# scientificcomputing/networks_fenicsx

Hardware: NVIDIA B200
Metric: tree-network assemble+solve DOFs/s (higher is better)
Workload: dtype f64

## Files before the change

networks_fenicsx_b200/csrc/ctx.cuh:

```cuda
#pragma once

#include <cuda_runtime.h>

#include <cstdarg>
#include <cstdint>
#include <cstdio>
#include <cstring>
#include <string>
#include <vector>

#include "../../include/nxfx_b200.h"

namespace nxfx {

constexpr int kTileRows = 256;
constexpr int kTileCap = 2048;
constexpr int kThreads = 256;

template <typename T>
struct DevBuf {
  T* p = nullptr;
  size_t n = 0;
  cudaError_t alloc(size_t count) {
    release();
// ... 72 lines not shown
  bool bottom_factored = false;
  int32_t n_nodes = 0, E = 0, gdim = 0, N = 0, n_bif = 0, n_inc = 0;
  int64_t nv = 0, nc = 0, nq = 0, poff = 0, loff = 0, ndofs = 0, nnz = 0;
  nxfx::DevBuf<double> x;
  nxfx::DevBuf<double> pos_stage;
  nxfx::DevBuf<int4> slot_uvl;
  nxfx::DevBuf<int2> slot_uv;
  nxfx::DevBuf<uint32_t> bif_in_bits;
  nxfx::DevBuf<int32_t> slot_edge, edge_slot, edge_u, edge_v, bif_ptr, bif_inc;
  nxfx::DevBuf<int32_t> rowptr, colidx, tile_base;
  bool pipe_ok = false;
  bool generic = false;
  nxfx::DevBuf<int32_t> gen_src_id, gen_bptr, gen_bid;
  nxfx::DevBuf<double> gen_src_coef, gen_bcoef, gen_cell_h;
  nxfx::Condensation cond;
  std::vector<nxfx::MatState*> mats;
  nxfx::MatState* cur = nullptr;
  int64_t next_mat_id = 1;
  bool pc_unscaled = false;
  int64_t pc_mat = -1;
  std::vector<int32_t> edge_slot_h;
  nxfx::TreeSchedule tree;
  nxfx::DevBuf<double> edge_g, edge_c, edge_fn;
  nxfx::DevBuf<double> work;
  nxfx::DevBuf<double> work2;
  nxfx::DevBuf<double> scal;
  nxfx::DevBuf<unsigned int> ticket;
  double* scal_h = nullptr;
  double* scal_h_dev = nullptr;
  bool pdl_coop_refused = false;
  int32_t n_shared = 0;
  nxfx::DevBuf<int32_t> shared_lm;
  std::vector<int32_t> shared_lm_h;
  nxfx::DevBuf<int32_t> top_sh_pos;
  nxfx::DevBuf<int32_t> top_sh_idx;
  nxfx::DevBuf<double> lam_weight, lam_nonshared;
  nxfx::DevBuf<double> p_nonshared;
  nxfx::PeerComm comm;
  double* mirror_h = nullptr;
  cudaStream_t side = nullptr;
  cudaEvent_t ev_x = nullptr;
  nxfx::DevBuf<double> e2e_pbc, e2e_b, e2e_x;
};

namespace nxfx {

// ... 34 lines not shown
```

networks_fenicsx_b200/csrc/nxfx_b200.cu:

```cuda

#include <cub/device/device_scan.cuh>

#include <algorithm>
#include <atomic>
#include <chrono>
#include <cmath>
#include <cstdlib>

#include "assemble.cuh"
#include "ctx.cuh"
#include "condense.cuh"
#include "generic.cuh"
#include "precond.cuh"
#include "spmv.cuh"

using namespace nxfx;

namespace {

constexpr int kScalPartials = 8 * kMaxPartials;
constexpr int kScalSlots = 1024;

Net make_net(const nxfx_ctx* c) {
  Net g;
// ... 227 lines not shown
  return NXFX_OK;
}

int do_residual(nxfx_ctx* ctx, const double* b, const double* x, double* r, double* norm2_d, bool pdl = false) {
  const int ntiles = (int)cdiv(ctx->ndofs, kTileRows);
  if (ctx->comm.ready) {
    NXFX_REQUIRE(ctx, ctx->pipe_ok && ctx->lam_nonshared.p, "the fused partitioned residual needs the pipelined SpMV and nxfx_set_shared");
    const int grid = std::min(ntiles, ctx->sm_count * kPipeBlocksPerSM);
    cudaLaunchConfig_t cfg = {};
    cfg.gridDim = dim3(grid);
    cfg.blockDim = dim3(kTileRows);
    cfg.dynamicSmemBytes = kPipeSmem;
    cfg.stream = ctx->stream;
    cudaLaunchAttribute attr[1];
    attr[0].id = cudaLaunchAttributeProgrammaticStreamSerialization;
    attr[0].val.programmaticStreamSerializationAllowed = 1;
    cfg.attrs = attr;
    cfg.numAttrs = pdl ? 1 : 0;
    NXFX_CUDA(ctx, cudaLaunchKernelEx(&cfg, spmv_pipe_kernel<3>, (int)ctx->ndofs, ntiles, (const int32_t*)ctx->rowptr.p,
                                      (const int32_t*)ctx->colidx.p, (const double*)ctx->cur->vals.p,
                                      (const int32_t*)ctx->tile_base.p, x, r, b, ctx->scal.p, ctx->ticket.p, norm2_d,
                                      (int)ctx->loff, (const double*)ctx->lam_nonshared.p, (const double*)ctx->lam_weight.p,
                                      make_peer(ctx, 1), (const int32_t*)ctx->shared_lm.p, (int)ctx->n_shared,
                                      ctx->comm.lam_scratch.p));
    ctx->launches++;
    return NXFX_OK;
  }
  if (ctx->pipe_ok && !pdl) {
    const int grid = std::min(ntiles, ctx->sm_count * kPipeBlocksPerSM);
    NXFX_LAUNCH(ctx, spmv_pipe_kernel<1>, grid, kTileRows, kPipeSmem, (int)ctx->ndofs, ntiles,
                ctx->rowptr.p, ctx->colidx.p, ctx->cur->vals.p, ctx->tile_base.p, x, r, b, ctx->scal.p,
                ctx->ticket.p, norm2_d);
    return NXFX_OK;
  }
  if (ctx->pipe_ok) {
    const int grid = std::min(ntiles, ctx->sm_count * kPipeBlocksPerSM);
    cudaLaunchConfig_t cfg = {};
    cfg.gridDim = dim3(grid);
    cfg.blockDim = dim3(kTileRows);
    cfg.dynamicSmemBytes = kPipeSmem;
    cfg.stream = ctx->stream;
    cudaLaunchAttribute attr[1];
    attr[0].id = cudaLaunchAttributeProgrammaticStreamSerialization;
    attr[0].val.programmaticStreamSerializationAllowed = 1;
    cfg.attrs = attr;
    cfg.numAttrs = 1;
    NXFX_CUDA(ctx, cudaLaunchKernelEx(&cfg, spmv_pipe_kernel<1>, (int)ctx->ndofs, ntiles, (const int32_t*)ctx->rowptr.p,
                                      (const int32_t*)ctx->colidx.p, (const double*)ctx->cur->vals.p,
                                      (const int32_t*)ctx->tile_base.p, x, r, b, ctx->scal.p, ctx->ticket.p, norm2_d, 0,
                                      (const double*)nullptr, (const double*)nullptr, PeerDev{}, (const int32_t*)nullptr, 0,
                                      (double*)nullptr));
    ctx->launches++;
    return NXFX_OK;
  }
  const int grid = std::min(ntiles, kMaxPartials);
  NXFX_LAUNCH(ctx, spmv_kernel<1>, grid, kTileRows, 0, (int)ctx->ndofs, ntiles, ctx->rowptr.p,
              ctx->colidx.p, ctx->cur->vals.p, x, r, b, ctx->scal.p, ctx->ticket.p, norm2_d);
  return NXFX_OK;
}

template <int K>
int launch_multi_dot(nxfx_ctx* ctx, int n, const double* A, size_t stride, const double* w, double* out) {
  NXFX_LAUNCH(ctx, multi_dot_kernel<K>, vec_grid(ctx, n), kThreads, 0, n, A, stride, w, ctx->scal.p,
              ctx->ticket.p, out);
  return NXFX_OK;
}

int do_multi_dot(nxfx_ctx* ctx, int n, int k, const double* A, size_t stride, const double* w, double* out) {
  int j = 0;
  while (j < k) {
    const int m = std::min(8, k - j);
    const double* Aj = A + (size_t)j * stride;
    int rc = NXFX_OK;
    switch (m) {
      case 8: rc = launch_multi_dot<8>(ctx, n, Aj, stride, w, out + j); break;
      case 7: rc = launch_multi_dot<7>(ctx, n, Aj, stride, w, out + j); break;
      case 6: rc = launch_multi_dot<6>(ctx, n, Aj, stride, w, out + j); break;
      case 5: rc = launch_multi_dot<5>(ctx, n, Aj, stride, w, out + j); break;
      case 4: rc = launch_multi_dot<4>(ctx, n, Aj, stride, w, out + j); break;
      case 3: rc = launch_multi_dot<3>(ctx, n, Aj, stride, w, out + j); break;
// ... 145 lines not shown

int cond_backward_local(nxfx_ctx* ctx, double* z, bool add) {
  Net g = make_net(ctx);
  CondDev c = make_cond(ctx);
  TreeDev t = make_tree(ctx);
  const int nb = ctx->tree.n_chunks - 1;
  if (ctx->n_bif > 0 && nb > 0) NXFX_LAUNCH(ctx, btree_sweep_kernel<2>, nb, 1024, 0, t, c, 0);
  const int grid = (int)cdiv((int64_t)ctx->E + ctx->n_bif, kCondThreads);
  if (add) NXFX_LAUNCH(ctx, cond_backsub_kernel<true>, grid, kCondThreads, 0, g, t, c, z);
  else NXFX_LAUNCH(ctx, cond_backsub_kernel<false>, grid, kCondThreads, 0, g, t, c, z);
  return NXFX_OK;
}

int do_cond_apply(nxfx_ctx* ctx, const double* r, double* z, bool add) {
  NXFX_REQUIRE(ctx, ctx->pc_ready, "pc_setup has not been run");
  int rc = cond_forward_local(ctx, r, nullptr);
  if (rc) return rc;
  if (ctx->n_bif > 0) NXFX_LAUNCH(ctx, btree_sweep_kernel<3>, 1, 1024, 0, make_tree(ctx), make_cond(ctx), ctx->tree.n_chunks - 1);
  return cond_backward_local(ctx, z, add);
}

bool n1_kernels(const nxfx_ctx* ctx) { return ctx->N == 1 && ctx->tree.fast_ok; }

int check_aligned(nxfx_ctx* ctx, const double* r, const double* z = nullptr) {
  NXFX_REQUIRE(ctx, (reinterpret_cast<uintptr_t>(r) & 15) == 0 && (reinterpret_cast<uintptr_t>(z) & 15) == 0,
               "vectors must be 16-byte aligned");
  return NXFX_OK;
}

int node_diag(nxfx_ctx* ctx, bool bif) {
  if (n1_kernels(ctx)) {
    if (bif) NXFX_LAUNCH(ctx, bif_diag_n1_kernel, (int)cdiv(ctx->n_bif, kThreads), kThreads, 0, make_net(ctx), make_tree(ctx), ctx->cur->cell_rh.p);
    return NXFX_OK;
  }
  NXFX_LAUNCH(ctx, edge_conductance_kernel, (int)cdiv(ctx->E, kThreads), kThreads, 0, ctx->E, ctx->N, ctx->cur->cell_rh.p, ctx->edge_g.p);
  if (bif) NXFX_LAUNCH(ctx, bif_diag_kernel, (int)cdiv(ctx->n_bif, kThreads), kThreads, 0, make_net(ctx), make_tree(ctx), ctx->edge_g.p);
  return NXFX_OK;
}

int node_rhs(nxfx_ctx* ctx, const double* r, bool bif) {
  Net g = make_net(ctx);
  TreeDev t = make_tree(ctx);
  if (n1_kernels(ctx)) {
    if (bif) NXFX_LAUNCH(ctx, bif_rhs_n1_kernel, (int)cdiv(ctx->n_bif, kThreads), kThreads, 0, g, t, r, ctx->cur->cell_rh.p, ctx->lam_weight.p);
    return NXFX_OK;
  }
  NXFX_LAUNCH(ctx, edge_condense_kernel<false>, (int)cdiv(ctx->E, kThreads), kThreads, 0, g, ctx->cur->cell_rh.p, r,
              ctx->edge_c.p, ctx->edge_fn.p, nullptr);
  if (bif)
    NXFX_LAUNCH(ctx, bif_rhs_kernel<false>, (int)cdiv(ctx->n_bif, kThreads), kThreads, 0, g, t, r, ctx->edge_g.p, ctx->edge_c.p,
                ctx->edge_fn.p, ctx->lam_weight.p);
  return NXFX_OK;
}

int edge_backsub(nxfx_ctx* ctx, const double* r, double* z, bool add, bool pdl = false) {
  Net g = make_net(ctx);
  TreeDev t = make_tree(ctx);
  const double* cell_rh = ctx->cur->cell_rh.p;
  const int grid = (int)cdiv((int64_t)ctx->E + ctx->n_bif, kThreads);
  if (!n1_kernels(ctx)) {
    if (add) NXFX_LAUNCH(ctx, edge_backsub_kernel<true>, grid, kThreads, 0, g, t, cell_rh, r, ctx->edge_g.p, ctx->edge_c.p, z);
    else NXFX_LAUNCH(ctx, edge_backsub_kernel<false>, grid, kThreads, 0, g, t, cell_rh, r, ctx->edge_g.p, ctx->edge_c.p, z);
    return NXFX_OK;
  }
  if (!pdl) {
    if (add) NXFX_LAUNCH(ctx, edge_backsub_n1_kernel<true>, grid, kThreads, 0, g, t, cell_rh, r, z);
    else NXFX_LAUNCH(ctx, edge_backsub_n1_kernel<false>, grid, kThreads, 0, g, t, cell_rh, r, z);
    return NXFX_OK;
  }
  cudaLaunchConfig_t cfg = {};
  cfg.gridDim = dim3((unsigned)grid);
  cfg.blockDim = dim3(kThreads);
  cfg.stream = ctx->stream;
  cudaLaunchAttribute attr[1];
  attr[0].id = cudaLaunchAttributeProgrammaticStreamSerialization;
  attr[0].val.programmaticStreamSerializationAllowed = 1;
  cfg.attrs = attr;
  cfg.numAttrs = 1;
  if (add) NXFX_CUDA(ctx, cudaLaunchKernelEx(&cfg, edge_backsub_n1_kernel<true>, g, t, cell_rh, r, z));
  else NXFX_CUDA(ctx, cudaLaunchKernelEx(&cfg, edge_backsub_n1_kernel<false>, g, t, cell_rh, r, z));
  ctx->launches++;
  return NXFX_OK;
}

int do_pc_setup(nxfx_ctx* ctx) {
  NXFX_REQUIRE(ctx, is_assembled(ctx), "assemble the matrix before pc_setup");
  if (ctx->generic) return do_cond_setup(ctx);
  NXFX_REQUIRE(ctx, ctx->tree.set, "nxfx_set_tree_schedule has not been called");
  const bool n1 = n1_kernels(ctx);
  int rc;
  if (!n1 && (rc = node_diag(ctx, ctx->n_bif > 0))) return rc;
  if (ctx->n_bif > 0 && (rc = tree_pass(ctx, true, nullptr, n1))) return rc;
  mark_factored(ctx);
  return NXFX_OK;
}

bool can_fuse_setup(const nxfx_ctx* ctx) {
  return !ctx->generic && ctx->tree.set && ctx->tree.fast_ok && ctx->tree.coop_fs_ok && ctx->n_bif > 0 &&
         ctx->tree.n_chunks > 1 && (!ctx->lam_weight.p || ctx->comm.ready) && ctx->cur->acc_count == 1;
}

int do_pc_setup_apply(nxfx_ctx* ctx, const double* r, double* z, bool add = false) {
  NXFX_REQUIRE(ctx, is_assembled(ctx), "assemble the matrix before pc_setup");
  const bool n1 = n1_kernels(ctx);
  if (n1) {
    int rc = check_aligned(ctx, r, z);
    if (rc) return rc;
  }
  auto& s = ctx->tree;
  Net g = make_net(ctx);
  TreeDev t = make_tree(ctx);
  FusedN1 fin{g, r, ctx->cur->cell_rh.p, ctx->lam_weight.p};
  unsigned int* tk = ctx->ticket.p + 1;
  unsigned int* fl = ctx->ticket.p + 2;
  unsigned int ep = ++s.epoch;
  int nb = s.n_chunks - 1;
  PeerDev pc = make_peer(ctx, 0);
  if (!n1) {
    NXFX_LAUNCH(ctx, edge_condense_kernel<true>, (int)cdiv(ctx->E, kThreads), kThreads, 0, g, ctx->cur->cell_rh.p, r,
                ctx->edge_c.p, ctx->edge_fn.p, ctx->edge_g.p);
    NXFX_LAUNCH(ctx, bif_rhs_kernel<true>, (int)cdiv(ctx->n_bif, kThreads), kThreads, 0, g, t, r, ctx->edge_g.p,
                ctx->edge_c.p, ctx->edge_fn.p, ctx->lam_weight.p);
    fin.r = nullptr;
    fin.cell_rh = nullptr;
  }
// ... 3 lines not shown
  cfg.blockDim = dim3(kTreeThreads);
  cfg.dynamicSmemBytes = tree_smem_bytes_fs(s.cap);
  cfg.stream = ctx->stream;
  cudaLaunchAttribute attr[2];
  attr[0].id = cudaLaunchAttributeCooperative;
  attr[0].val.cooperative = 1;
  attr[1].id = cudaLaunchAttributeProgrammaticStreamSerialization;
  attr[1].val.programmaticStreamSerializationAllowed = 1;
  cfg.attrs = attr;
  cfg.numAttrs = ctx->pdl_coop_refused ? 1 : 2;
  const bool multi = gb < nb;
  auto kern = pc.nranks > 1 ? (multi ? tree_factor_solve_coop_kernel<true, true> : tree_factor_solve_coop_kernel<true, false>)
                            : (multi ? tree_factor_solve_coop_kernel<false, true> : tree_factor_solve_coop_kernel<false, false>);
  cudaError_t le = cudaLaunchKernelEx(&cfg, kern, t, nb, tk, fl, ep, fin, pc);
  if (le != cudaSuccess && cfg.numAttrs == 2) {
    cudaGetLastError();
    ctx->pdl_coop_refused = true;
    cfg.numAttrs = 1;
    le = cudaLaunchKernelEx(&cfg, kern, t, nb, tk, fl, ep, fin, pc);
  }
  NXFX_CUDA(ctx, le);
  ctx->launches++;
  mark_factored(ctx);
  return edge_backsub(ctx, r, z, add, true);
}

int do_pc_apply(nxfx_ctx* ctx, int pc_type, const double* r, double* z, bool add = false) {
  const int n = (int)ctx->ndofs;
  if (pc_type == NXFX_PC_NETWORK_SCHUR && ctx->cur->acc_count > 1 && !ctx->pc_unscaled) {
    const size_t ld = vec_stride(ctx);
    if (ctx->work2.n < 2 * ld) {
      NXFX_CUDA(ctx, cudaStreamSynchronize(ctx->stream));
      NXFX_CUDA(ctx, ctx->work2.alloc(2 * ld));
    }
    const double inv_k = 1.0 / (double)ctx->cur->acc_count;
    double* rs = ctx->work2.p;
    double* zs = ctx->work2.p + ld;
    NXFX_LAUNCH(ctx, scale_tail_kernel<false>, vec_grid(ctx, n), kThreads, 0, n, (int)ctx->poff, inv_k, r, rs);
    ctx->pc_unscaled = true;
    const int rc = do_pc_apply(ctx, pc_type, rs, zs, false);
    ctx->pc_unscaled = false;
    if (rc) return rc;
    if (add) NXFX_LAUNCH(ctx, scale_tail_kernel<true>, vec_grid(ctx, n), kThreads, 0, n, (int)ctx->poff, inv_k, zs, z);
    else NXFX_LAUNCH(ctx, scale_tail_kernel<false>, vec_grid(ctx, n), kThreads, 0, n, (int)ctx->poff, inv_k, zs, z);
    return NXFX_OK;
  }
  if (add && pc_type != NXFX_PC_NETWORK_SCHUR) {
    int rc = ensure_work(ctx, 3);
    if (rc) return rc;
    double* tmp = ctx->work.p + 2 * vec_stride(ctx);
// ... 3 lines not shown
  }
  if (ctx->comm.ready) {
    NXFX_REQUIRE(ctx, pc_type == NXFX_PC_NETWORK_SCHUR && can_fuse_setup(ctx),
                 "the fused partitioned solve needs a forest schedule that fits the cooperative kernel and pc_type lu");
    return do_pc_setup_apply(ctx, r, z, add);
  }
  if (pc_type == NXFX_PC_NONE) {
    NXFX_CUDA(ctx, cudaMemcpyAsync(z, r, n * sizeof(double), cudaMemcpyDeviceToDevice, ctx->stream));
    return NXFX_OK;
  }
  if (pc_type == NXFX_PC_JACOBI_FLUX) {
    NXFX_LAUNCH(ctx, jacobi_flux_kernel, (int)cdiv(n, kThreads), kThreads, 0, n, (int)ctx->nq,
                ctx->rowptr.p, ctx->colidx.p, ctx->cur->vals.p, r, z);
    return NXFX_OK;
  }
  NXFX_REQUIRE(ctx, ctx->pc_ready, "pc_setup has not been run");
  if (ctx->generic) return do_cond_apply(ctx, r, z, add);
  const bool n1 = n1_kernels(ctx);
  int rc;
  if (n1 && (rc = check_aligned(ctx, r, z))) return rc;
  const bool fuse = n1 && ctx->n_bif > 0 && ctx->tree.coop_ok && ctx->tree.n_chunks > 1 && !ctx->lam_weight.p;
  if ((rc = node_rhs(ctx, r, ctx->n_bif > 0 && !fuse))) return rc;
  if (ctx->n_bif > 0 && (rc = tree_pass(ctx, false, r, fuse))) return rc;
  return edge_backsub(ctx, r, z, add);
}

int factor_bottom(nxfx_ctx* ctx) {
  if (ctx->generic) return cond_factor_local(ctx);
  int rc = node_diag(ctx, true);
  if (rc) return rc;
  const int nb = ctx->tree.n_chunks - 1;
  if (nb > 0) NXFX_LAUNCH(ctx, tree_factor_kernel, nb, kTreeThreads, tree_smem_bytes(ctx->tree.cap), make_tree(ctx), nb, ctx->ticket.p + 1, 0,
                          (FusedN1{make_net(ctx), nullptr, nullptr}));
  return NXFX_OK;
}

int forward_bottom(nxfx_ctx* ctx, const double* r) {
  if (ctx->generic) return cond_forward_local(ctx, r, ctx->lam_weight.p);
  int rc = node_rhs(ctx, r, true);
  if (rc) return rc;
  const int nb = ctx->tree.n_chunks - 1;
  if (nb > 0) NXFX_LAUNCH(ctx, tree_solve_kernel<kTreeUp>, nb, kTreeThreads, tree_smem_bytes(ctx->tree.cap), make_tree(ctx), nb, ctx->ticket.p + 1, 0);
  return NXFX_OK;
}

template <bool FACTOR, int PHASE>
int top_split(nxfx_ctx* ctx, double* buf) {
// ... 54 lines not shown
bool poll_norms_enabled() {
  static const bool on = [] { const char* e = std::getenv("NXFX_POLL_NORMS"); return !(e && e[0] == '0'); }();
  return on;
}

void push_history(nxfx_solve_info* info, double v) {
  if (info->history_len < NXFX_HISTORY_LEN) info->history[info->history_len++] = v;
}

int mirror_copy(nxfx_ctx* ctx, const double* x) {
  if (!ctx->mirror_h) return NXFX_OK;
  NXFX_CUDA(ctx, cudaEventRecord(ctx->ev_x, ctx->stream));
  NXFX_CUDA(ctx, cudaStreamWaitEvent(ctx->side, ctx->ev_x, 0));
  NXFX_CUDA(ctx, cudaMemcpyAsync(ctx->mirror_h, x, (size_t)ctx->ndofs * sizeof(double), cudaMemcpyDeviceToHost, ctx->side));
  return NXFX_OK;
}

int solve_preonly(nxfx_ctx* ctx, const double* b, double* x, const nxfx_solve_opts* o, nxfx_solve_info* info,
                  bool fused_setup) {
  int rc = ensure_work(ctx, 3);
  if (rc) return rc;
  double* r = ctx->work.p;
  const int steps = std::max(0, std::min(o->refine_steps, 32));
  if ((rc = fused_setup ? do_pc_setup_apply(ctx, b, x) : do_pc_apply(ctx, o->pc_type, b, x, false))) return rc;
  if ((rc = mirror_copy(ctx, x))) return rc;
  info->iterations = 1;
  if (steps == 0 && !o->final_residual) {
    NXFX_CUDA(ctx, cudaStreamSynchronize(ctx->stream));
    info->rhs_norm = info->residual_norm = -1.0;
    info->converged = 1;
    return NXFX_OK;
  }
  const double rt = o->refine_rtol > 0.0 ? o->refine_rtol : 0.0;
  int applied = 0;
  while (true) {
    const bool lazy = ctx->pipe_ok;
    volatile double* nh = ctx->scal_h;
    const bool poll = poll_norms_enabled();
    if (poll) { ctx->scal_h[0] = kNormSentinel(); ctx->scal_h[1] = kNormSentinel(); }
    if ((rc = do_residual(ctx, b, x, lazy ? nullptr : r, ctx->scal_h_dev, true))) return rc;
    bool arrived = false;
    if (poll) {
      const auto t0 = std::chrono::steady_clock::now();
      for (unsigned spin = 0;; ++spin) {
        if (!is_norm_sentinel(nh[0]) && !is_norm_sentinel(nh[1])) { arrived = true; break; }
        if ((spin & 255u) == 255u && std::chrono::steady_clock::now() - t0 > std::chrono::microseconds(1500)) break;
      }
      std::atomic_thread_fence(std::memory_order_acquire);
    }
    if (!arrived) NXFX_CUDA(ctx, cudaStreamSynchronize(ctx->stream));
    info->rhs_norm = std::sqrt(ctx->scal_h[1]);
    info->residual_norm = std::sqrt(ctx->scal_h[0]);
    push_history(info, info->residual_norm);
    const bool good = std::isfinite(info->residual_norm) && info->residual_norm <= rt * info->rhs_norm;
    if (applied >= steps || (good && rt > 0.0) || !std::isfinite(info->residual_norm)) break;
    if (lazy && (rc = do_residual(ctx, b, x, r, slot(ctx, 0)))) return rc;
    if ((rc = do_pc_apply(ctx, o->pc_type, r, x, true))) return rc;
    if ((rc = mirror_copy(ctx, x))) return rc;
    ++applied;
    if (applied >= steps && !o->final_residual) break;
  }
  info->iterations = 1 + applied;
  const double tol = std::max(o->rtol * info->rhs_norm, o->atol);
// ... 79 lines not shown
    }
  }
  info->iterations = its;
  info->converged = std::isfinite(info->residual_norm) && info->residual_norm <= tol;
  return NXFX_OK;
}

int setup_spmv_tiles(nxfx_ctx* ctx) {
  const int n = (int)ctx->ndofs;
  const int ntiles = (int)cdiv(n, kTileRows);
  NXFX_CUDA(ctx, ctx->tile_base.alloc((size_t)ntiles + 2));
  int32_t* max_tile = reinterpret_cast<int32_t*>(ctx->ticket.p);
  NXFX_LAUNCH(ctx, tile_base_kernel, (int)cdiv(ntiles + 1, kThreads), kThreads, 0, n, ntiles, ctx->rowptr.p,
              ctx->tile_base.p, max_tile);
  int32_t max_tile_h = 0;
  NXFX_CUDA(ctx, cudaMemcpyAsync(&max_tile_h, max_tile, sizeof(int32_t), cudaMemcpyDeviceToHost, ctx->stream));
  NXFX_CUDA(ctx, cudaMemsetAsync(ctx->ticket.p, 0, sizeof(unsigned int), ctx->stream));
  NXFX_CUDA(ctx, cudaStreamSynchronize(ctx->stream));
  ctx->pipe_ok = max_tile_h + 8 <= kPipeCap;
  if (ctx->pipe_ok) {
    NXFX_CUDA(ctx, cudaFuncSetAttribute(spmv_pipe_kernel<0>, cudaFuncAttributeMaxDynamicSharedMemorySize, (int)kPipeSmem));
    NXFX_CUDA(ctx, cudaFuncSetAttribute(spmv_pipe_kernel<1>, cudaFuncAttributeMaxDynamicSharedMemorySize, (int)kPipeSmem));
    NXFX_CUDA(ctx, cudaFuncSetAttribute(spmv_pipe_kernel<2>, cudaFuncAttributeMaxDynamicSharedMemorySize, (int)kPipeSmem));
  }
  return NXFX_OK;
}

}

extern "C" {

int nxfx_abi_version(void) { return NXFX_ABI_VERSION; }

int nxfx_create(nxfx_ctx** out, int device) {
  if (!out) return NXFX_ERR_INVALID;
  *out = nullptr;
  int count = 0;
  cudaError_t e = cudaGetDeviceCount(&count);
  if (e != cudaSuccess || device < 0 || device >= count) return NXFX_ERR_CUDA;
  if (cudaSetDevice(device) != cudaSuccess) return NXFX_ERR_CUDA;
  auto* ctx = new nxfx_ctx();
  ctx->device = device;
  cudaDeviceProp prop;
  if (cudaGetDeviceProperties(&prop, device) == cudaSuccess) ctx->sm_count = prop.multiProcessorCount;
  cudaEventCreate(&ctx->ev0);
  cudaEventCreate(&ctx->ev1);
// ... 137 lines not shown
  int rc;
  if ((rc = upload(ctx, ctx->pos_stage, node_pos, (size_t)n_nodes * gdim))) return rc;
  if ((rc = upload(ctx, ctx->edge_u, edge_u, (size_t)E))) return rc;
  if ((rc = upload(ctx, ctx->edge_v, edge_v, (size_t)E))) return rc;
  if ((rc = upload(ctx, ctx->edge_slot, edge_slot, (size_t)E))) return rc;
  if ((rc = upload(ctx, ctx->slot_edge, slot_edge.data(), (size_t)E))) return rc;
  if ((rc = upload(ctx, ctx->slot_uvl, uvl.data(), (size_t)E))) return rc;
  std::vector<int2> uv((size_t)E);
  for (int64_t s = 0; s < E; ++s) uv[s] = make_int2(uvl[s].x, uvl[s].y);
  if ((rc = upload(ctx, ctx->slot_uv, uv.data(), (size_t)E))) return rc;
  std::vector<uint32_t> in_bits((size_t)(n_inc + 31) / 32 + 1, 0u);
  for (int32_t k = 0; k < n_inc; ++k)
    if (bif_inc[k] & 1) in_bits[k >> 5] |= 1u << (k & 31);
  if ((rc = upload(ctx, ctx->bif_in_bits, in_bits.data(), in_bits.size()))) return rc;
  DevBuf<int32_t> node_lm_d;
  if ((rc = upload(ctx, node_lm_d, node_lm, (size_t)n_nodes))) return rc;
  if ((rc = upload(ctx, ctx->bif_ptr, bif_ptr, (size_t)n_bif + 1))) return rc;
  if ((rc = upload(ctx, ctx->bif_inc, bif_inc, (size_t)n_inc))) return rc;
  NXFX_CUDA(ctx, ctx->x.alloc((size_t)nv * 4));
  NXFX_CUDA(ctx, cudaMemsetAsync(ctx->x.p, 0, (size_t)nv * 4 * sizeof(double), ctx->stream));
  NXFX_CUDA(ctx, ctx->edge_g.alloc((size_t)E));
  NXFX_CUDA(ctx, ctx->edge_c.alloc((size_t)E));
  NXFX_CUDA(ctx, ctx->edge_fn.alloc((size_t)E));
  if ((rc = ensure_scal(ctx))) return rc;
  if ((rc = build_vertices(ctx))) return rc;
  NXFX_LAUNCH(ctx, tag_lm_kernel, (int)cdiv(n_nodes, kThreads), kThreads, 0, n_nodes, node_lm_d.p, ctx->x.p);
  NXFX_CUDA(ctx, cudaStreamSynchronize(ctx->stream));
  ctx->has_network = true;
  return NXFX_OK;
}

int nxfx_update_node_positions(nxfx_ctx* ctx, const double* node_pos) {
  if (!ctx) return NXFX_ERR_INVALID;
  NXFX_REQUIRE(ctx, ctx->has_network && node_pos, "no network / null input");
  NXFX_CUDA(ctx, cudaMemcpyAsync(ctx->pos_stage.p, node_pos, (size_t)ctx->n_nodes * ctx->gdim * sizeof(double),
                                 cudaMemcpyHostToDevice, ctx->stream));
  return build_vertices(ctx);
}

int nxfx_get_sizes(const nxfx_ctx* ctx, int64_t* nv, int64_t* nc, int64_t* ndofs, int64_t* nnz) {
  if (!ctx || !ctx->has_network) return NXFX_ERR_INVALID;
  if (nv) *nv = ctx->nv;
  if (nc) *nc = ctx->nc;
  if (ndofs) *ndofs = ctx->ndofs;
  if (nnz) *nnz = ctx->nnz;
  return NXFX_OK;
// ... 804 lines not shown
```

networks_fenicsx_b200/csrc/precond.cuh:

```cuda
#pragma once

#include "assemble.cuh"
#include "peer.cuh"
#include "spmv.cuh"

namespace nxfx {

struct TreeDev {
  const int32_t* __restrict__ t_of_bif;
  const int32_t* __restrict__ bif_of_t;
  const int32_t* __restrict__ t_parent;
  const int32_t* __restrict__ t_pedge;
  const int32_t* __restrict__ t_pslot;
  const int32_t* __restrict__ t_cptr;
  const int32_t* __restrict__ t_cidx;
  const int32_t* __restrict__ chunk_lptr;
  const int32_t* __restrict__ lvl_ptr;
  const int32_t* __restrict__ chunk_desc;
  const int32_t* __restrict__ t_inc_ptr;
  const int2* __restrict__ t_inc;
  double* diag0;
  double* tg;
  double* d;
  double* gd;
// ... 1078 lines not shown
  const int n = t.t_of_bif[i];
  t.diag0[n] = s;
  const int pe = t.t_pslot[n];
  t.tg[n] = pe >= 0 ? 1.0 / cell_rh[pe] : 0.0;
}

__global__ void __launch_bounds__(kThreads)
bif_rhs_n1_kernel(Net g, TreeDev t, const double* __restrict__ r, const double* __restrict__ cell_rh,
                  const double* __restrict__ lam_weight) {
  const int i = blockIdx.x * blockDim.x + threadIdx.x;
  if (i >= g.n_bif) return;
  double s = lam_weight ? -lam_weight[i] * r[g.loff + i] : -r[g.loff + i];
  for (int k = g.bif_ptr[i]; k < g.bif_ptr[i + 1]; ++k) {
    const int inc = g.bif_inc[k], e = inc >> 1;
    const int slot = g.edge_slot[e];
    const double2 rq = *reinterpret_cast<const double2*>(r + 2 * (size_t)slot);
    const double rp = r[g.poff + e], rh = cell_rh[slot];
    const double gc = (1.0 / rh) * (rq.x + rq.y) - 0.5 * rp;
    s += (inc & 1) ? (rp + gc) : -gc;
  }
  t.r[t.t_of_bif[i]] = s;
}

template <bool ADD>
__global__ void __launch_bounds__(kThreads)
edge_backsub_n1_kernel(Net g, TreeDev t, const double* __restrict__ cell_rh, const double* __restrict__ r,
                       double* __restrict__ z) {
  asm volatile("griddepcontrol.launch_dependents;");
  const int idx = blockIdx.x * blockDim.x + threadIdx.x;
  if (idx >= g.E) {
    asm volatile("griddepcontrol.wait;" ::: "memory");
    const int i = idx - g.E;
    if (i < g.n_bif) { if (ADD) z[g.loff + i] += t.lam_nat[i]; else z[g.loff + i] = t.lam_nat[i]; }
    return;
  }
  const int slot = idx;
  const int4 uv = g.slot_uvl[slot];
  const int e = g.slot_edge[slot];
  const double2 rq = *reinterpret_cast<const double2*>(r + 2 * (size_t)slot);
  const double rp = r[g.poff + e], rh = cell_rh[slot];
  asm volatile("griddepcontrol.wait;" ::: "memory");
  const double lu = uv.z >= 0 ? t.lam_nat[uv.z] : 0.0;
  const double lv = uv.w >= 0 ? t.lam_nat[uv.w] : 0.0;
  const double c = (rq.x + rq.y) - 0.5 * rh * rp;
  const double q0 = (c + lu - lv) / rh;
  const double q1 = q0 + rp;
  const double p = lu + rq.x - rh * (q0 * kThird + q1 * kSixth);
  double2* zq = reinterpret_cast<double2*>(z + 2 * (size_t)slot);
  if (ADD) {
    const double2 o = *zq;
    *zq = make_double2(o.x + q0, o.y + q1);
    z[g.poff + e] += p;
  } else {
    *zq = make_double2(q0, q1);
    z[g.poff + e] = p;
  }
}

__global__ void __launch_bounds__(kThreads)
pack_shared_kernel(int n_shared, int loff, const int32_t* __restrict__ shared_lm,
                   const double* __restrict__ v, double* __restrict__ buf) {
  const int i = blockIdx.x * blockDim.x + threadIdx.x;
  if (i < n_shared) buf[i] = v[loff + shared_lm[i]];
}

__global__ void __launch_bounds__(kThreads)
residual_finish_kernel(int n_shared, int loff, const int32_t* __restrict__ shared_lm,
                       const double* __restrict__ buf, double* __restrict__ r, double* __restrict__ nrm_out) {
  __shared__ double red[kThreads / 32];
  double acc = 0.0;
  for (int i = threadIdx.x; i < n_shared; i += blockDim.x) {
    const double v = buf[i];
    r[loff + shared_lm[i]] = v;
    acc += v * v;
  }
  acc = warp_sum(acc);
  if ((threadIdx.x & 31) == 0) red[threadIdx.x >> 5] = acc;
  __syncthreads();
// ... 24 lines not shown
```

networks_fenicsx_b200/csrc/spmv.cuh:

```cuda
#pragma once

#include "ctx.cuh"
#include "peer.cuh"

namespace nxfx {

constexpr int kEntriesPerThread = kTileCap / kTileRows;
constexpr int kMaxPartials = 4096;

__device__ __forceinline__ double warp_sum(double v) {
#pragma unroll
  for (int o = 16; o > 0; o >>= 1) v += __shfl_down_sync(0xffffffffu, v, o);
  return v;
}

template <int THREADS>
__device__ __forceinline__ double block_sum(double v, double* red ) {
  v = warp_sum(v);
  const int lane = threadIdx.x & 31, w = threadIdx.x >> 5;
  if (lane == 0) red[w] = v;
  __syncthreads();
  double s = 0.0;
  if (w == 0) {
    s = lane < THREADS / 32 ? red[lane] : 0.0;
    s = warp_sum(s);
  }
  __syncthreads();
  return s;
}

template <int THREADS, int K>
__device__ __forceinline__ bool finish_partials(double (&mine)[K], double* partial, int nblocks,
                                                unsigned int* ticket, double* out, double* red) {
  __shared__ bool last;
  if (threadIdx.x == 0) {
#pragma unroll
    for (int k = 0; k < K; ++k) partial[(size_t)k * kMaxPartials + blockIdx.x] = mine[k];
    __threadfence();
    const unsigned int t = atomicAdd(ticket, 1u);
    last = (t == (unsigned int)nblocks - 1);
  }
  __syncthreads();
  if (!last) return false;
  __threadfence();
#pragma unroll
  for (int k = 0; k < K; ++k) {
    double s = 0.0;
    for (int i = threadIdx.x; i < nblocks; i += THREADS)
      s += ((volatile double*)partial)[(size_t)k * kMaxPartials + i];
    s = block_sum<THREADS>(s, red);
    if (threadIdx.x == 0) out[k] = s;
  }
  if (threadIdx.x == 0) *ticket = 0u;
  return true;
}

template <int MODE>
__global__ void __launch_bounds__(kTileRows)
spmv_kernel(int n, int ntiles, const int32_t* __restrict__ rowptr,
            const int32_t* __restrict__ colidx, const double* __restrict__ vals,
            const double* __restrict__ x, double* __restrict__ y, const double* __restrict__ b,
            double* partial, unsigned int* ticket, double* norm2_out) {
  __shared__ double sm[kTileCap];
  __shared__ int srow[kTileRows + 1];
  __shared__ double red[kTileRows / 32];
  double nrm = 0.0, nrb = 0.0;
  for (int tile = blockIdx.x; tile < ntiles; tile += gridDim.x) {
    const int r0 = tile * kTileRows;
    const int nr = min(kTileRows, n - r0);
    if (threadIdx.x <= nr) srow[threadIdx.x] = rowptr[r0 + threadIdx.x];
// ... 93 lines not shown
  }
}

__global__ void __launch_bounds__(kThreads)
tile_base_kernel(int n, int ntiles, const int32_t* __restrict__ rowptr, int32_t* __restrict__ tile_base,
                 int32_t* __restrict__ max_tile_nnz) {
  const int t = blockIdx.x * blockDim.x + threadIdx.x;
  if (t > ntiles) return;
  const int r = min(t * kTileRows, n);
  const int b = rowptr[r];
  tile_base[t] = b;
  if (t < ntiles) atomicMax(max_tile_nnz, rowptr[min(r + kTileRows, n)] - b);
}

template <int MODE>
__global__ void __launch_bounds__(kTileRows)
spmv_pipe_kernel(int n, int ntiles, const int32_t* __restrict__ rowptr,
                 const int32_t* __restrict__ colidx, const double* __restrict__ vals,
                 const int32_t* __restrict__ tile_base, const double* __restrict__ x,
                 double* __restrict__ y, const double* __restrict__ b, double* partial,
                 unsigned int* ticket, double* norm2_out, int loff = 0,
                 const double* __restrict__ w_r = nullptr, const double* __restrict__ w_b = nullptr,
                 PeerDev pc = PeerDev{}, const int32_t* __restrict__ shared_lm = nullptr, int n_shared = 0,
                 double* lam_scratch = nullptr) {
  extern __shared__ __align__(128) unsigned char smem_raw[];
  SpmvStage* st = reinterpret_cast<SpmvStage*>(smem_raw);
  uint64_t* full = reinterpret_cast<uint64_t*>(smem_raw + kStages * sizeof(SpmvStage));
  __shared__ double red[kTileRows / 32];
  const int tid = threadIdx.x;
  if (tid == 0) {
    for (int s = 0; s < kStages; ++s) mbar_init(full + s, 1);
    asm volatile("fence.mbarrier_init.release.cluster;" ::: "memory");
    asm volatile("fence.proxy.async.shared::cta;" ::: "memory");
  }
  __syncthreads();
  const uint64_t stream_policy = l2_evict_first_policy();
  auto issue = [&](int tile, int s) {
    const int r0 = tile * kTileRows;
    const int nr = min(kTileRows, n - r0);
    const int sb = tile_base[tile], se = tile_base[tile + 1];
    const int s4 = sb & ~3;
    const int cnt4 = ((se + 3) & ~3) - s4;
    const uint32_t rbytes = (uint32_t)(((nr + 1) * 4 + 15) & ~15);
    mbar_expect_tx(full + s, (uint32_t)cnt4 * 12u + rbytes);
    if (cnt4 > 0) {
      bulk_g2s_stream(st[s].vals, vals + s4, (uint32_t)cnt4 * 8u, full + s, stream_policy);
      bulk_g2s_stream(st[s].cols, colidx + s4, (uint32_t)cnt4 * 4u, full + s, stream_policy);
    }
    bulk_g2s_stream(st[s].rows, rowptr + r0, rbytes, full + s, stream_policy);
  };
  if (tid == 0) {
    for (int k = 0; k < kStages - 1; ++k) {
      const int tile = blockIdx.x + k * gridDim.x;
      if (tile < ntiles) issue(tile, k);
    }
  }
  asm volatile("griddepcontrol.wait;" ::: "memory");
  double nrm = 0.0, nrb = 0.0;
  int it = 0;
  for (int tile = blockIdx.x; tile < ntiles; tile += gridDim.x, ++it) {
    const int s = it % kStages;
    if (tid == 0) {
      const int pre = tile + (kStages - 1) * gridDim.x;
      if (pre < ntiles) {
        asm volatile("fence.proxy.async.shared::cta;" ::: "memory");
        issue(pre, (it + kStages - 1) % kStages);
      }
    }
    const int r0 = tile * kTileRows;
    const int nr = min(kTileRows, n - r0);
    double bi = 0.0;
    if (MODE >= 1 && tid < nr) bi = __ldcs(b + r0 + tid);
    mbar_wait(full + s, (uint32_t)((it / kStages) & 1));
    SpmvStage& S = st[s];
    const int base = S.rows[0];
    const int off = base & 3;
    const int tnnz = S.rows[nr] - base;
    constexpr int kPer = kPipeCap / kTileRows;
    int c[kPer];
    double xv[kPer];
#pragma unroll
    for (int k = 0; k < kPer; ++k) {
      const int idx = tid + k * kTileRows;
      if (idx < tnnz) c[k] = S.cols[off + idx];
    }
#pragma unroll
    for (int k = 0; k < kPer; ++k) {
      const int idx = tid + k * kTileRows;
      if (idx < tnnz) xv[k] = x[c[k]];
    }
#pragma unroll
    for (int k = 0; k < kPer; ++k) {
      const int idx = tid + k * kTileRows;
      if (idx < tnnz) S.vals[off + idx] = __dmul_rn(S.vals[off + idx], xv[k]);
    }
    __syncthreads();
    if (tid < nr) {
      const int rs = S.rows[tid] - base + off, re = S.rows[tid + 1] - base + off;
      double acc = 0.0;
      for (int k = rs; k < re; ++k) acc = __dadd_rn(acc, S.vals[k]);
      if (MODE == 0) {
        y[r0 + tid] = acc;
      } else {
        const double r = __dsub_rn(bi, acc);
        if (y) y[r0 + tid] = r;
        if (MODE >= 2 && r0 + tid >= loff) {
          const double wr = w_r[r0 + tid - loff];
          nrm += wr * r * r;
          nrb += w_b[r0 + tid - loff] * bi * bi;
          if (MODE == 3 && wr == 0.0) lam_scratch[r0 + tid - loff] = r;
        } else {
          nrm += r * r;
          nrb += bi * bi;
        }
      }
    }
    asm volatile("fence.proxy.async.shared::cta;" ::: "memory");
    __syncthreads();
  }
  if (MODE >= 1 && MODE < 3) {
    double mine[2] = {block_sum<kTileRows>(nrm, red), block_sum<kTileRows>(nrb, red)};
    finish_partials<kTileRows, 2>(mine, partial, gridDim.x, ticket, norm2_out, red);
  }
  if (MODE == 3) {
    __shared__ double loc[2];
    double mine[2] = {block_sum<kTileRows>(nrm, red), block_sum<kTileRows>(nrb, red)};
    if (!finish_partials<kTileRows, 2>(mine, partial, gridDim.x, ticket, loc, red)) return;
    __syncthreads();
    peer_ll_send(pc, 1, n_shared + 2,
                 [&](int i) { return i < n_shared ? __ldcg(lam_scratch + shared_lm[i]) : loc[i - n_shared]; });
    double acc = 0.0;
    for (int i = tid; i < n_shared; i += kTileRows) {
      double v = 0.0;
      for (int src = 0; src < pc.nranks; ++src) v += peer_ll_recv(pc, 1, src, i);
      if (y) y[loff + shared_lm[i]] = v;
      acc += v * v;
    }
    acc = block_sum<kTileRows>(acc, red);
    if (tid == 0) {
      double s0 = acc, s1 = 0.0;
      for (int src = 0; src < pc.nranks; ++src) {
        s0 += peer_ll_recv(pc, 1, src, n_shared);
        s1 += peer_ll_recv(pc, 1, src, n_shared + 1);
      }
      norm2_out[0] = s0;
// ... 82 lines not shown
```

Baseline: 21.35 billion.

## Fuse edge residual into N=1 back-substitution and run SpMV only on multiplier rows

For the network Schur preconditioner with N=1 and the tree fast path, the edge back-substitution kernel now also computes the residual of the flux and pressure rows it has just produced. It prefetches the matrix values for its rows into shared memory with cp.async and writes per-block partial norms. The residual step then launches a new SpMV mode that covers only tiles from the multiplier offset onward and folds in those partials. This skips a second read of x, the colidx and the row pointers for the edge rows, at the cost of a specialised kernel that assumes a fixed per-row layout of five or fewer nonzeros.

```diff
diff --git a/networks_fenicsx_b200/csrc/ctx.cuh b/networks_fenicsx_b200/csrc/ctx.cuh
--- a/networks_fenicsx_b200/csrc/ctx.cuh
+++ b/networks_fenicsx_b200/csrc/ctx.cuh
@@ -118,6 +118,7 @@
   std::vector<int32_t> edge_slot_h;
   nxfx::TreeSchedule tree;
   nxfx::DevBuf<double> edge_g, edge_c, edge_fn;
+  nxfx::DevBuf<double> flux_part;
   nxfx::DevBuf<double> work;
   nxfx::DevBuf<double> work2;
   nxfx::DevBuf<double> scal;
diff --git a/networks_fenicsx_b200/csrc/nxfx_b200.cu b/networks_fenicsx_b200/csrc/nxfx_b200.cu
--- a/networks_fenicsx_b200/csrc/nxfx_b200.cu
+++ b/networks_fenicsx_b200/csrc/nxfx_b200.cu
@@ -273,7 +273,7 @@
                                       (const int32_t*)ctx->tile_base.p, x, r, b, ctx->scal.p, ctx->ticket.p, norm2_d,
                                       (int)ctx->loff, (const double*)ctx->lam_nonshared.p, (const double*)ctx->lam_weight.p,
                                       make_peer(ctx, 1), (const int32_t*)ctx->shared_lm.p, (int)ctx->n_shared,
-                                      ctx->comm.lam_scratch.p));
+                                      ctx->comm.lam_scratch.p, (const double*)nullptr, 0));
     ctx->launches++;
     return NXFX_OK;
   }
@@ -300,13 +300,36 @@
                                       (const int32_t*)ctx->colidx.p, (const double*)ctx->cur->vals.p,
                                       (const int32_t*)ctx->tile_base.p, x, r, b, ctx->scal.p, ctx->ticket.p, norm2_d, 0,
                                       (const double*)nullptr, (const double*)nullptr, PeerDev{}, (const int32_t*)nullptr, 0,
-                                      (double*)nullptr));
+                                      (double*)nullptr, (const double*)nullptr, 0));
     ctx->launches++;
     return NXFX_OK;
   }
   const int grid = std::min(ntiles, kMaxPartials);
   NXFX_LAUNCH(ctx, spmv_kernel<1>, grid, kTileRows, 0, (int)ctx->ndofs, ntiles, ctx->rowptr.p,
               ctx->colidx.p, ctx->cur->vals.p, x, r, b, ctx->scal.p, ctx->ticket.p, norm2_d);
+  return NXFX_OK;
+}
+
+int do_residual_rest(nxfx_ctx* ctx, const double* b, const double* x, double* norm2_d, int row0) {
+  const int ntiles = (int)cdiv(ctx->ndofs, kTileRows);
+  const int grid = std::max(1, std::min(ntiles - row0 / kTileRows, ctx->sm_count * kPipeBlocksPerSM));
+  cudaLaunchConfig_t cfg = {};
+  cfg.gridDim = dim3(grid);
+  cfg.blockDim = dim3(kTileRows);
+  cfg.dynamicSmemBytes = kPipeSmem;
+  cfg.stream = ctx->stream;
+  cudaLaunchAttribute attr[1];
+  attr[0].id = cudaLaunchAttributeProgrammaticStreamSerialization;
+  attr[0].val.programmaticStreamSerializationAllowed = 1;
+  cfg.attrs = attr;
+  cfg.numAttrs = 1;
+  NXFX_CUDA(ctx, cudaLaunchKernelEx(&cfg, spmv_pipe_kernel<4>, (int)ctx->ndofs, ntiles, (const int32_t*)ctx->rowptr.p,
+                                    (const int32_t*)ctx->colidx.p, (const double*)ctx->cur->vals.p,
+                                    (const int32_t*)ctx->tile_base.p, x, (double*)nullptr, b, ctx->scal.p, ctx->ticket.p,
+                                    norm2_d, row0, (const double*)nullptr, (const double*)nullptr, PeerDev{},
+                                    (const int32_t*)nullptr, 0, (double*)nullptr, (const double*)ctx->flux_part.p,
+                                    (int)cdiv(ctx->E, kThreads)));
+  ctx->launches++;
   return NXFX_OK;
 }
 
@@ -498,6 +521,11 @@
 
 bool n1_kernels(const nxfx_ctx* ctx) { return ctx->N == 1 && ctx->tree.fast_ok; }
 
+bool split_residual(const nxfx_ctx* ctx, int pc_type) {
+  return pc_type == NXFX_PC_NETWORK_SCHUR && !ctx->generic && n1_kernels(ctx) && ctx->pipe_ok && !ctx->comm.ready &&
+         !ctx->lam_weight.p && ctx->cur->acc_count == 1;
+}
+
 int check_aligned(nxfx_ctx* ctx, const double* r, const double* z = nullptr) {
   NXFX_REQUIRE(ctx, (reinterpret_cast<uintptr_t>(r) & 15) == 0 && (reinterpret_cast<uintptr_t>(z) & 15) == 0,
                "vectors must be 16-byte aligned");
@@ -529,11 +557,26 @@
   return NXFX_OK;
 }
 
-int edge_backsub(nxfx_ctx* ctx, const double* r, double* z, bool add, bool pdl = false) {
+int edge_backsub(nxfx_ctx* ctx, const double* r, double* z, bool add, bool pdl = false, bool resid = false) {
   Net g = make_net(ctx);
   TreeDev t = make_tree(ctx);
   const double* cell_rh = ctx->cur->cell_rh.p;
   const int grid = (int)cdiv((int64_t)ctx->E + ctx->n_bif, kThreads);
+  if (resid) {
+    cudaLaunchConfig_t cfg = {};
+    cfg.gridDim = dim3((unsigned)grid);
+    cfg.blockDim = dim3(kThreads);
+    cfg.stream = ctx->stream;
+    cudaLaunchAttribute attr[1];
+    attr[0].id = cudaLaunchAttributeProgrammaticStreamSerialization;
+    attr[0].val.programmaticStreamSerializationAllowed = 1;
+    cfg.attrs = attr;
+    cfg.numAttrs = pdl ? 1 : 0;
+    NXFX_CUDA(ctx, cudaLaunchKernelEx(&cfg, edge_backsub_resid_n1_kernel, g, t, cell_rh, r, z, (const int32_t*)ctx->rowptr.p,
+                                      (const double*)ctx->cur->vals.p, ctx->flux_part.p));
+    ctx->launches++;
+    return NXFX_OK;
+  }
   if (!n1_kernels(ctx)) {
     if (add) NXFX_LAUNCH(ctx, edge_backsub_kernel<true>, grid, kThreads, 0, g, t, cell_rh, r, ctx->edge_g.p, ctx->edge_c.p, z);
     else NXFX_LAUNCH(ctx, edge_backsub_kernel<false>, grid, kThreads, 0, g, t, cell_rh, r, ctx->edge_g.p, ctx->edge_c.p, z);
@@ -576,7 +619,7 @@
          ctx->tree.n_chunks > 1 && (!ctx->lam_weight.p || ctx->comm.ready) && ctx->cur->acc_count == 1;
 }
 
-int do_pc_setup_apply(nxfx_ctx* ctx, const double* r, double* z, bool add = false) {
+int do_pc_setup_apply(nxfx_ctx* ctx, const double* r, double* z, bool add = false, bool resid = false) {
   NXFX_REQUIRE(ctx, is_assembled(ctx), "assemble the matrix before pc_setup");
   const bool n1 = n1_kernels(ctx);
   if (n1) {
@@ -626,10 +669,10 @@
   NXFX_CUDA(ctx, le);
   ctx->launches++;
   mark_factored(ctx);
-  return edge_backsub(ctx, r, z, add, true);
-}
-
-int do_pc_apply(nxfx_ctx* ctx, int pc_type, const double* r, double* z, bool add = false) {
+  return edge_backsub(ctx, r, z, add, true, resid);
+}
+
+int do_pc_apply(nxfx_ctx* ctx, int pc_type, const double* r, double* z, bool add = false, bool resid = false) {
   const int n = (int)ctx->ndofs;
   if (pc_type == NXFX_PC_NETWORK_SCHUR && ctx->cur->acc_count > 1 && !ctx->pc_unscaled) {
     const size_t ld = vec_stride(ctx);
@@ -679,7 +722,7 @@
   const bool fuse = n1 && ctx->n_bif > 0 && ctx->tree.coop_ok && ctx->tree.n_chunks > 1 && !ctx->lam_weight.p;
   if ((rc = node_rhs(ctx, r, ctx->n_bif > 0 && !fuse))) return rc;
   if (ctx->n_bif > 0 && (rc = tree_pass(ctx, false, r, fuse))) return rc;
-  return edge_backsub(ctx, r, z, add);
+  return edge_backsub(ctx, r, z, add, false, resid);
 }
 
 int factor_bottom(nxfx_ctx* ctx) {
@@ -780,7 +823,9 @@
   if (rc) return rc;
   double* r = ctx->work.p;
   const int steps = std::max(0, std::min(o->refine_steps, 32));
-  if ((rc = fused_setup ? do_pc_setup_apply(ctx, b, x) : do_pc_apply(ctx, o->pc_type, b, x, false))) return rc;
+  const bool split = (steps > 0 || o->final_residual) && split_residual(ctx, o->pc_type);
+  if ((rc = fused_setup ? do_pc_setup_apply(ctx, b, x, false, split) : do_pc_apply(ctx, o->pc_type, b, x, false, split)))
+    return rc;
   if ((rc = mirror_copy(ctx, x))) return rc;
   info->iterations = 1;
   if (steps == 0 && !o->final_residual) {
@@ -796,7 +841,9 @@
     volatile double* nh = ctx->scal_h;
     const bool poll = poll_norms_enabled();
     if (poll) { ctx->scal_h[0] = kNormSentinel(); ctx->scal_h[1] = kNormSentinel(); }
-    if ((rc = do_residual(ctx, b, x, lazy ? nullptr : r, ctx->scal_h_dev, true))) return rc;
+    if (split && applied == 0) rc = do_residual_rest(ctx, b, x, ctx->scal_h_dev, (int)ctx->loff);
+    else rc = do_residual(ctx, b, x, lazy ? nullptr : r, ctx->scal_h_dev, true);
+    if (rc) return rc;
     bool arrived = false;
     if (poll) {
       const auto t0 = std::chrono::steady_clock::now();
@@ -922,6 +969,7 @@
     NXFX_CUDA(ctx, cudaFuncSetAttribute(spmv_pipe_kernel<0>, cudaFuncAttributeMaxDynamicSharedMemorySize, (int)kPipeSmem));
     NXFX_CUDA(ctx, cudaFuncSetAttribute(spmv_pipe_kernel<1>, cudaFuncAttributeMaxDynamicSharedMemorySize, (int)kPipeSmem));
     NXFX_CUDA(ctx, cudaFuncSetAttribute(spmv_pipe_kernel<2>, cudaFuncAttributeMaxDynamicSharedMemorySize, (int)kPipeSmem));
+    NXFX_CUDA(ctx, cudaFuncSetAttribute(spmv_pipe_kernel<4>, cudaFuncAttributeMaxDynamicSharedMemorySize, (int)kPipeSmem));
   }
   return NXFX_OK;
 }
@@ -1105,6 +1153,7 @@
   NXFX_CUDA(ctx, ctx->edge_g.alloc((size_t)E));
   NXFX_CUDA(ctx, ctx->edge_c.alloc((size_t)E));
   NXFX_CUDA(ctx, ctx->edge_fn.alloc((size_t)E));
+  NXFX_CUDA(ctx, ctx->flux_part.alloc(2 * (size_t)cdiv(E, kThreads)));
   if ((rc = ensure_scal(ctx))) return rc;
   if ((rc = build_vertices(ctx))) return rc;
   NXFX_LAUNCH(ctx, tag_lm_kernel, (int)cdiv(n_nodes, kThreads), kThreads, 0, n_nodes, node_lm_d.p, ctx->x.p);
diff --git a/networks_fenicsx_b200/csrc/precond.cuh b/networks_fenicsx_b200/csrc/precond.cuh
--- a/networks_fenicsx_b200/csrc/precond.cuh
+++ b/networks_fenicsx_b200/csrc/precond.cuh
@@ -1124,6 +1124,16 @@
   t.r[t.t_of_bif[i]] = s;
 }
 
+struct EdgeN1 {
+  double q0, q1, p;
+};
+__device__ __forceinline__ EdgeN1 edge_unknowns_n1(double2 rq, double rp, double rh, double lu, double lv) {
+  const double c = (rq.x + rq.y) - 0.5 * rh * rp;
+  const double q0 = (c + lu - lv) / rh;
+  const double q1 = q0 + rp;
+  return EdgeN1{q0, q1, lu + rq.x - rh * (q0 * kThird + q1 * kSixth)};
+}
+
 template <bool ADD>
 __global__ void __launch_bounds__(kThreads)
 edge_backsub_n1_kernel(Net g, TreeDev t, const double* __restrict__ cell_rh, const double* __restrict__ r,
@@ -1144,18 +1154,112 @@
   asm volatile("griddepcontrol.wait;" ::: "memory");
   const double lu = uv.z >= 0 ? t.lam_nat[uv.z] : 0.0;
   const double lv = uv.w >= 0 ? t.lam_nat[uv.w] : 0.0;
-  const double c = (rq.x + rq.y) - 0.5 * rh * rp;
-  const double q0 = (c + lu - lv) / rh;
-  const double q1 = q0 + rp;
-  const double p = lu + rq.x - rh * (q0 * kThird + q1 * kSixth);
+  const EdgeN1 u = edge_unknowns_n1(rq, rp, rh, lu, lv);
   double2* zq = reinterpret_cast<double2*>(z + 2 * (size_t)slot);
   if (ADD) {
     const double2 o = *zq;
-    *zq = make_double2(o.x + q0, o.y + q1);
-    z[g.poff + e] += p;
+    *zq = make_double2(o.x + u.q0, o.y + u.q1);
+    z[g.poff + e] += u.p;
   } else {
-    *zq = make_double2(q0, q1);
-    z[g.poff + e] = p;
+    *zq = make_double2(u.q0, u.q1);
+    z[g.poff + e] = u.p;
+  }
+}
+
+__device__ __forceinline__ void cp_async16(void* dst, const void* src) {
+  asm volatile("cp.async.cg.shared.global [%0], [%1], 16;" ::"r"(smem_u32(dst)), "l"(src) : "memory");
+}
+
+__global__ void __launch_bounds__(kThreads)
+edge_backsub_resid_n1_kernel(Net g, TreeDev t, const double* __restrict__ cell_rh, const double* __restrict__ b,
+                             double* __restrict__ x, const int32_t* __restrict__ rowptr,
+                             const double* __restrict__ vals, double* __restrict__ partial) {
+  __shared__ __align__(16) double sm[kAsmCap + 2];
+  __shared__ int warp_nl[kThreads / 32];
+  __shared__ double red[kThreads / 32];
+  asm volatile("griddepcontrol.launch_dependents;");
+  const int idx = blockIdx.x * blockDim.x + threadIdx.x;
+  const int nsb = (g.E + kThreads - 1) / kThreads;
+  if ((int)blockIdx.x >= nsb) {
+    asm volatile("griddepcontrol.wait;" ::: "memory");
+    const int i = idx - g.E;
+    if (i < g.n_bif) x[g.loff + i] = t.lam_nat[i];
+    return;
+  }
+  const int r0 = 2 * kThreads * blockIdx.x;
+  const int sbase = rowptr[r0], send = rowptr[min(r0 + 2 * kThreads, g.nq)];
+  {
+    const int s2 = sbase & ~1;
+    const int npair = (send - s2 + 1) >> 1;
+    for (int q = threadIdx.x; q < npair; q += kThreads) cp_async16(sm + 2 * q, vals + s2 + 2 * q);
+    asm volatile("cp.async.commit_group;" ::: "memory");
+  }
+  const int slot = idx;
+  const bool active = slot < g.E;
+  int4 uv = make_int4(0, 0, -1, -1);
+  int e = 0;
+  double2 rq = make_double2(0.0, 0.0), pv = make_double2(0.0, 0.0);
+  double rp = 0.0, rh = 1.0;
+  if (active) {
+    uv = g.slot_uvl[slot];
+    e = g.slot_edge[slot];
+    rq = *reinterpret_cast<const double2*>(b + 2 * (size_t)slot);
+    rp = b[g.poff + e];
+    rh = cell_rh[slot];
+    pv = *reinterpret_cast<const double2*>(vals + rowptr[g.poff] + 2 * (size_t)e);
+  }
+  const bool hu = uv.z >= 0, hv = uv.w >= 0;
+  const int lane = threadIdx.x & 31, w = threadIdx.x >> 5;
+  const unsigned bu = __ballot_sync(0xffffffffu, hu), bv = __ballot_sync(0xffffffffu, hv);
+  const unsigned lt = (1u << lane) - 1u;
+  int pre = __popc(bu & lt) + __popc(bv & lt);
+  if (lane == 0) warp_nl[w] = __popc(bu) + __popc(bv);
+  asm volatile("griddepcontrol.wait;" ::: "memory");
+  double nrm = 0.0, nrb = 0.0;
+  EdgeN1 u{0.0, 0.0, 0.0};
+  double lu = 0.0, lv = 0.0;
+  if (active) {
+    lu = hu ? t.lam_nat[uv.z] : 0.0;
+    lv = hv ? t.lam_nat[uv.w] : 0.0;
+    u = edge_unknowns_n1(rq, rp, rh, lu, lv);
+    *reinterpret_cast<double2*>(x + 2 * (size_t)slot) = make_double2(u.q0, u.q1);
+    x[g.poff + e] = u.p;
+  } else {
+    const int i = idx - g.E;
+    if (i < g.n_bif) x[g.loff + i] = t.lam_nat[i];
+  }
+  asm volatile("cp.async.wait_all;" ::: "memory");
+  __syncthreads();
+#pragma unroll
+  for (int k = 0; k < kThreads / 32; ++k)
+    if (k < w) pre += warp_nl[k];
+  if (active) {
+    const int nl = (int)hu + (int)hv;
+    const bool ufirst = !hv || (hu && uv.z < uv.w);
+    const double la = ufirst ? lu : lv, lb = ufirst ? lv : lu;
+    auto row = [&](const double* v, double bi) {
+      double acc = __dadd_rn(0.0, __dmul_rn(v[0], u.q0));
+      acc = __dadd_rn(acc, __dmul_rn(v[1], u.q1));
+      acc = __dadd_rn(acc, __dmul_rn(v[2], u.p));
+      if (nl > 0) acc = __dadd_rn(acc, __dmul_rn(v[3], la));
+      if (nl > 1) acc = __dadd_rn(acc, __dmul_rn(v[4], lb));
+      const double r = __dsub_rn(bi, acc);
+      nrm += r * r;
+      nrb += bi * bi;
+    };
+    const double* v0 = sm + (sbase & 1) + 6 * (int)threadIdx.x + 2 * pre;
+    row(v0, rq.x);
+    row(v0 + 3 + nl, rq.y);
+    const double acc = __dadd_rn(__dadd_rn(0.0, __dmul_rn(pv.x, u.q0)), __dmul_rn(pv.y, u.q1));
+    const double r = __dsub_rn(rp, acc);
+    nrm += r * r;
+    nrb += rp * rp;
+  }
+  const double s_r = block_sum<kThreads>(nrm, red);
+  const double s_b = block_sum<kThreads>(nrb, red);
+  if (threadIdx.x == 0) {
+    partial[blockIdx.x] = s_r;
+    partial[nsb + blockIdx.x] = s_b;
   }
 }
 
diff --git a/networks_fenicsx_b200/csrc/spmv.cuh b/networks_fenicsx_b200/csrc/spmv.cuh
--- a/networks_fenicsx_b200/csrc/spmv.cuh
+++ b/networks_fenicsx_b200/csrc/spmv.cuh
@@ -31,7 +31,8 @@
 
 template <int THREADS, int K>
 __device__ __forceinline__ bool finish_partials(double (&mine)[K], double* partial, int nblocks,
-                                                unsigned int* ticket, double* out, double* red) {
+                                                unsigned int* ticket, double* out, double* red,
+                                                const double* pre = nullptr, int npre = 0) {
   __shared__ bool last;
   if (threadIdx.x == 0) {
 #pragma unroll
@@ -46,6 +47,7 @@
 #pragma unroll
   for (int k = 0; k < K; ++k) {
     double s = 0.0;
+    for (int i = threadIdx.x; i < npre; i += THREADS) s += pre[(size_t)k * npre + i];
     for (int i = threadIdx.x; i < nblocks; i += THREADS)
       s += ((volatile double*)partial)[(size_t)k * kMaxPartials + i];
     s = block_sum<THREADS>(s, red);
@@ -185,7 +187,7 @@
                  unsigned int* ticket, double* norm2_out, int loff = 0,
                  const double* __restrict__ w_r = nullptr, const double* __restrict__ w_b = nullptr,
                  PeerDev pc = PeerDev{}, const int32_t* __restrict__ shared_lm = nullptr, int n_shared = 0,
-                 double* lam_scratch = nullptr) {
+                 double* lam_scratch = nullptr, const double* __restrict__ pre = nullptr, int n_pre = 0) {
   extern __shared__ __align__(128) unsigned char smem_raw[];
   SpmvStage* st = reinterpret_cast<SpmvStage*>(smem_raw);
   uint64_t* full = reinterpret_cast<uint64_t*>(smem_raw + kStages * sizeof(SpmvStage));
@@ -212,16 +214,17 @@
     }
     bulk_g2s_stream(st[s].rows, rowptr + r0, rbytes, full + s, stream_policy);
   };
+  const int tile0 = MODE == 4 ? loff / kTileRows : 0;
   if (tid == 0) {
     for (int k = 0; k < kStages - 1; ++k) {
-      const int tile = blockIdx.x + k * gridDim.x;
+      const int tile = tile0 + blockIdx.x + k * gridDim.x;
       if (tile < ntiles) issue(tile, k);
     }
   }
   asm volatile("griddepcontrol.wait;" ::: "memory");
   double nrm = 0.0, nrb = 0.0;
   int it = 0;
-  for (int tile = blockIdx.x; tile < ntiles; tile += gridDim.x, ++it) {
+  for (int tile = tile0 + blockIdx.x; tile < ntiles; tile += gridDim.x, ++it) {
     const int s = it % kStages;
     if (tid == 0) {
       const int pre = tile + (kStages - 1) * gridDim.x;
@@ -232,8 +235,9 @@
     }
     const int r0 = tile * kTileRows;
     const int nr = min(kTileRows, n - r0);
+    const bool counted = tid < nr && (MODE != 4 || r0 + tid >= loff);
     double bi = 0.0;
-    if (MODE >= 1 && tid < nr) bi = __ldcs(b + r0 + tid);
+    if (MODE >= 1 && counted) bi = __ldcs(b + r0 + tid);
     mbar_wait(full + s, (uint32_t)((it / kStages) & 1));
     SpmvStage& S = st[s];
     const int base = S.rows[0];
@@ -258,7 +262,7 @@
       if (idx < tnnz) S.vals[off + idx] = __dmul_rn(S.vals[off + idx], xv[k]);
     }
     __syncthreads();
-    if (tid < nr) {
+    if (counted) {
       const int rs = S.rows[tid] - base + off, re = S.rows[tid + 1] - base + off;
       double acc = 0.0;
       for (int k = rs; k < re; ++k) acc = __dadd_rn(acc, S.vals[k]);
@@ -267,7 +271,7 @@
       } else {
         const double r = __dsub_rn(bi, acc);
         if (y) y[r0 + tid] = r;
-        if (MODE >= 2 && r0 + tid >= loff) {
+        if ((MODE == 2 || MODE == 3) && r0 + tid >= loff) {
           const double wr = w_r[r0 + tid - loff];
           nrm += wr * r * r;
           nrb += w_b[r0 + tid - loff] * bi * bi;
@@ -281,9 +285,9 @@
     asm volatile("fence.proxy.async.shared::cta;" ::: "memory");
     __syncthreads();
   }
-  if (MODE >= 1 && MODE < 3) {
+  if (MODE == 1 || MODE == 2 || MODE == 4) {
     double mine[2] = {block_sum<kTileRows>(nrm, red), block_sum<kTileRows>(nrb, red)};
-    finish_partials<kTileRows, 2>(mine, partial, gridDim.x, ticket, norm2_out, red);
+    finish_partials<kTileRows, 2>(mine, partial, gridDim.x, ticket, norm2_out, red, pre, n_pre);
   }
   if (MODE == 3) {
     __shared__ double loc[2];
```

Result: no change. 21.48 billion, median of 6 (+0.6%).
